# nerficg-project/faster-gaussian-splatting

Hardware: AMD Instinct MI355X
Metric: train_iters_per_sec (higher is better)
Workload: dtype f32; 1 GPU; S2: 3000000 garden-like Gaussians (SH degree 3), 1920x1080, 8 orbit views; full training iteration fwd+loss+bwd+Adam (BASELINE.json configs[2]), loss 0.8*L1+0.2*DSSIM, densification_info updated; parallelism=single GPU, n_gaussians=3000000, active_sh_bases=16, forward=one host read per pass (fgs_forward), world=1, backend=none (single process), device=cuda:0 (AMD Radeon Graphics)

## Files before the change

### faster-gaussian-splatting_amd/FasterGSCudaBackend/__init__.py

```python
from ._lib import ExtensionError, library

library()

from ._backend import RasterizerSettings
from .rasterization import (async_forward_scope, async_forward_stats, diff_rasterize, diff_rasterize_aux, live_block_stats, rasterize, rasterize_aux, set_async_forward,
                            set_live_block_handover, take_async_overflow, update_pruning_scores)
from .adam import FusedAdam
from .fused import FusedRasterizerOptimizer


from .aux_ops import add_noise, relocation_adjustment, update_3d_filter

__all__ = ['diff_rasterize', 'diff_rasterize_aux', 'rasterize', 'rasterize_aux', 'update_pruning_scores', 'RasterizerSettings', 'FusedAdam', 'update_3d_filter',
           'relocation_adjustment', 'add_noise', 'FusedRasterizerOptimizer', 'ExtensionError', 'set_async_forward', 'async_forward_stats',
           'set_live_block_handover', 'live_block_stats', 'take_async_overflow', 'async_forward_scope']
```

### faster-gaussian-splatting_amd/FasterGSCudaBackend/_backend.py

```python
from __future__ import annotations

import ctypes as C
from typing import NamedTuple, Optional, Sequence

import torch

from . import _lib


class RasterizerSettings(NamedTuple):
    w2c: torch.Tensor
    cam_position: torch.Tensor
    bg_color: torch.Tensor
    active_sh_bases: int
    width: int
    height: int
    focal_x: float
    focal_y: float
    center_x: float
    center_y: float
    near_plane: float
    far_plane: float
    proper_antialiasing: bool

# ... 191 lines not shown
        return image

    def inference_aux(self, means, scales, rotations, opacities, sh0, sh_rest, settings: RasterizerSettings, to_chw: bool,
                      clamp_output: bool, alpha: bool = True, depth_expected: bool = True, depth_median: bool = True) -> dict:
        device, S, keep, buffers, cb, st = self._forward_setup((means, scales, rotations, opacities, sh0, sh_rest), settings)
        shape = (3, settings.height, settings.width) if to_chw else (settings.height, settings.width, 3)
        out = {'rgb': torch.empty(shape, dtype=torch.float32, device=device)}
        for name, wanted in (('alpha', alpha), ('depth', depth_expected), ('depth_median', depth_median)):
            if wanted:
                out[name] = torch.empty((settings.height, settings.width), dtype=torch.float32, device=device)
        maps = [out[k].data_ptr() if k in out else None for k in ('alpha', 'depth', 'depth_median')]
        self._check(self.lib.fgs_inference_aux(_ptr(means), _ptr(scales), _ptr(rotations), _ptr(opacities), _ptr(sh0), _ptr(sh_rest),
                                               means.shape[0], C.byref(S), out['rgb'].data_ptr(), int(to_chw), int(clamp_output), *maps, cb, None,
                                               C.byref(st), _stream_of(device)), 'fgs_inference_aux')
        return out

    def pruning_scores(self, scores, means, scales, rotations, opacities, sh0, sh_rest, settings: RasterizerSettings) -> None:
        device = self._check_params((scores, means, scales, rotations, opacities, sh0, sh_rest), ('scores',) + PARAMETER_NAMES)
        if scores.numel() != means.shape[0]:
            raise RuntimeError('scores must have one entry per Gaussian')
        S, keep, buffers, cb, st = self._forward_state(settings, total_sh_rest(sh_rest), device)
        self._check(self.lib.fgs_pruning_scores(_ptr(scores), _ptr(means), _ptr(scales), _ptr(rotations), _ptr(opacities), _ptr(sh0),
                                                _ptr(sh_rest), means.shape[0], C.byref(S), cb, None, C.byref(st), _stream_of(device)),
                    'fgs_pruning_scores')

    def _scratch(self, n: int, settings: RasterizerSettings, device: torch.device) -> torch.Tensor:
        return _empty_bytes(self.lib.fgs_backward_scratch_bytes(n, int(settings.width), int(settings.height)), device)

    def _scratch_aux(self, n: int, settings: RasterizerSettings, device: torch.device) -> torch.Tensor:
        return _empty_bytes(self.lib.fgs_backward_aux_scratch_bytes(n, int(settings.width), int(settings.height)), device)

    def backward(self, densification_info, grad_image, image, means, scales, rotations, opacities, sh_rest, buffers, settings,
                 state, out: tuple | None = None, live_blocks: Optional[torch.Tensor] = None,
                 reached_blocks: Optional[torch.Tensor] = None) -> tuple:
        return self.backward_aux(densification_info, grad_image, None, None, image, None, means, scales, rotations, opacities, sh_rest, buffers, settings,
                                 state, out, live_blocks, reached_blocks)

    def backward_aux(self, densification_info, grad_image, grad_alpha, grad_depth, image, depth, means, scales, rotations, opacities, sh_rest,
                     buffers, settings, state, out: tuple | None = None, live_blocks: Optional[torch.Tensor] = None,
                     reached_blocks: Optional[torch.Tensor] = None) -> tuple:
        aux = grad_alpha is not None or grad_depth is not None
        device = self._check_params((means, scales, rotations, opacities, sh_rest), BACKWARD_PARAMETER_NAMES)
        keep: list = []
        n = means.shape[0]
        total_rest = total_sh_rest(sh_rest)
        S = self._settings(settings, total_rest, device, keep)
        grad_image = grad_image.to(dtype=torch.float32).contiguous()
        if aux:
            hw = (int(settings.height), int(settings.width))
            for name, t in (('grad_alpha', grad_alpha), ('grad_depth', grad_depth), ('depth', depth if grad_depth is not None else None)):
                if t is not None and (tuple(t.shape) != hw or t.device != device):
                    raise RuntimeError(f'{name} must be a [H,W] = {hw} tensor on the parameters\' device')
            if grad_depth is not None and depth is None:
                raise RuntimeError('backward_aux: grad_depth needs the expected-depth map of forward_aux')
            grad_alpha = grad_alpha.to(dtype=torch.float32).contiguous() if grad_alpha is not None else None
            grad_depth = grad_depth.to(dtype=torch.float32).contiguous() if grad_depth is not None else None
        depth = depth.to(dtype=torch.float32).contiguous() if grad_depth is not None else None
        grads = _gradients_out(out, gradient_shapes(n, total_rest), device)
        dens = _densification(densification_info, n, device, validate=True)
        _check_block_flags('live_blocks', live_blocks, n, device)
        _check_block_flags('reached_blocks', reached_blocks, n, device)
        scratch = (self._scratch_aux if aux else self._scratch)(n, settings, device)
        st = _lib.ForwardState(*state)
        self._check(self.lib.fgs_backward_reached(_ptr(grad_image), _ptr(image), _ptr(grad_alpha), _ptr(grad_depth), _ptr(depth), _ptr(means), _ptr(scales),
                                                  _ptr(rotations), _ptr(opacities), _ptr(sh_rest), _ptr(buffers[0]), _ptr(buffers[1]), _ptr(buffers[2]),
                                                  _ptr(buffers[3]), _ptr(grads[0]), _ptr(grads[1]), _ptr(grads[2]), _ptr(grads[3]), _ptr(grads[4]), _ptr(grads[5]),
                                                  _ptr(dens), scratch.data_ptr(), n, C.byref(S), C.byref(st), _ptr(live_blocks), _ptr(reached_blocks),
                                                  _stream_of(device)),
                    'fgs_backward_aux' if aux else 'fgs_backward')
        return grads

    def backward_adam_fused(self, densification_info, grad_image, image, params: Sequence[torch.Tensor], exp_avgs, exp_avg_sqs,
                            buffers, settings, state, step: int, lrs: Sequence[float], betas=(0.9, 0.999), eps: float = 1e-15,
                            grad_alpha=None, grad_depth=None) -> None:
        if grad_alpha is not None or grad_depth is not None:
            raise RuntimeError('backward_adam_fused takes no alpha / depth gradients: use backward_aux and an optimizer step of its own')
        device = self._check_params(tuple(params) + tuple(exp_avgs) + tuple(exp_avg_sqs), ['param/moment'] * 18)
        keep: list = []
        n = params[0].shape[0]
        S = self._settings(settings, total_sh_rest(params[2]), device, keep)
        grad_image = grad_image.to(dtype=torch.float32).contiguous()
        dens = _densification(densification_info, n, device, validate=False)
        scratch = self._scratch(n, settings, device)
        st = _lib.ForwardState(*state)
        lr_arr = (C.c_double * 6)(*[float(x) for x in lrs])
        self._check(self.lib.fgs_backward_adam_fused(_ptr(grad_image), _ptr(image), _pointer_array(params, 6), _pointer_array(exp_avgs, 6),
                                                     _pointer_array(exp_avg_sqs, 6), _ptr(buffers[0]), _ptr(buffers[1]), _ptr(buffers[2]),
                                                     _ptr(buffers[3]), _ptr(dens), scratch.data_ptr(), n, C.byref(S), C.byref(st), int(step), lr_arr,
                                                     float(betas[0]), float(betas[1]), float(eps), _stream_of(device)),
                    'fgs_backward_adam_fused')

    def adam_step(self, grad, param, exp_avg, exp_avg_sq, step: int, lr: float, beta1: float, beta2: float, eps: float) -> None:
        device = self._check_params((grad, param, exp_avg, exp_avg_sq), ('param_grad', 'param', 'exp_avg', 'exp_avg_sq'))
        self._check(self.lib.fgs_adam_step(_ptr(grad), _ptr(param), _ptr(exp_avg), _ptr(exp_avg_sq), param.numel(), int(step),
                                           float(lr), float(beta1), float(beta2), float(eps), _stream_of(device)), 'fgs_adam_step')

    def adam_step_multi(self, grads, params, exp_avgs, exp_avg_sqs, steps, lrs, beta1: float, beta2: float, eps: float,
                        live_blocks: Optional[torch.Tensor] = None, quiet_blocks: Optional[torch.Tensor] = None) -> None:
        k = len(params)
        if k == 0:
            return
# ... 277 lines not shown
```

### faster-gaussian-splatting_amd/FasterGSCudaBackend/_lib.py

```python
from __future__ import annotations

import ctypes as C
import os
from pathlib import Path

PACKAGE_ROOT = Path(__file__).resolve().parent.parent
DEFAULT_LIBRARY = PACKAGE_ROOT / 'libfgs_hip.so'

FGS_BUF_PRIMITIVE, FGS_BUF_TILE, FGS_BUF_INSTANCE, FGS_BUF_BUCKET, FGS_BUF_SCRATCH = 0, 1, 2, 3, 4


class ExtensionError(ImportError):
    """Counterpart of Framework.ExtensionError raised by the reference's package init."""


class Settings(C.Structure):
    _fields_ = [
        ('w2c', C.c_void_p), ('cam_position', C.c_void_p), ('bg_color', C.c_void_p),
        ('active_sh_bases', C.c_int32), ('total_sh_bases_rest', C.c_int32), ('width', C.c_int32), ('height', C.c_int32),
        ('focal_x', C.c_float), ('focal_y', C.c_float), ('center_x', C.c_float), ('center_y', C.c_float),
        ('near_plane', C.c_float), ('far_plane', C.c_float), ('proper_antialiasing', C.c_int32),
    ]


class ForwardState(C.Structure):
    _fields_ = [('n_visible', C.c_int32), ('n_instances', C.c_int32), ('n_buckets', C.c_int32), ('selector', C.c_int32)]


class StageTime(C.Structure):
    _fields_ = [('name', C.c_char_p), ('total_ms', C.c_double), ('calls', C.c_int64)]


class BlobEntry(C.Structure):
    _fields_ = [('name', C.c_char_p), ('offset', C.c_size_t), ('bytes', C.c_size_t)]


SPLAT_RECORD_BYTES, ACC_RECORD_BYTES = 56, 36

RESIZE_FN = C.CFUNCTYPE(C.c_void_p, C.c_void_p, C.c_int32, C.c_size_t)

_P, _I32, _I64, _F64 = C.c_void_p, C.c_int32, C.c_int64, C.c_double

_SIGNATURES = {
    'fgs_abi_version': (C.c_int32, []),
    'fgs_last_error': (C.c_char_p, []),
    'fgs_build_info': (C.c_char_p, []),
    'fgs_forward': (C.c_int32, [_P] * 6 + [_I32, C.POINTER(Settings), _P, RESIZE_FN, _P, C.POINTER(ForwardState), _P]),
    'fgs_forward_aux': (C.c_int32, [_P] * 6 + [_I32, C.POINTER(Settings), _P, _P, _P, RESIZE_FN, _P, C.POINTER(ForwardState), _P]),
    'fgs_backward_aux_scratch_bytes': (C.c_size_t, [_I32, _I32, _I32]),
    'fgs_backward_aux': (C.c_int32, [_P] * 5 + [_P] * 5 + [_P] * 4 + [_P] * 6 + [_P, _P, _I32, C.POINTER(Settings), C.POINTER(ForwardState), _P, _P]),
    'fgs_backward_reached': (C.c_int32, [_P] * 5 + [_P] * 5 + [_P] * 4 + [_P] * 6 + [_P, _P, _I32, C.POINTER(Settings), C.POINTER(ForwardState), _P, _P, _P]),
    'fgs_forward_async': (C.c_int32, [_P] * 6 + [_I32, C.POINTER(Settings), _P, _I32, RESIZE_FN, _P, C.POINTER(ForwardState), _P]),
    'fgs_forward_counts': (C.c_int32, [_P, _I32, _P, _P]),
    'fgs_backward_scratch_bytes': (C.c_size_t, [_I32, _I32, _I32]),
    'fgs_backward': (C.c_int32, [_P] * 2 + [_P] * 5 + [_P] * 4 + [_P] * 6 + [_P, _P, _I32, C.POINTER(Settings), C.POINTER(ForwardState), _P]),
    'fgs_backward_live': (C.c_int32, [_P] * 2 + [_P] * 5 + [_P] * 4 + [_P] * 6 + [_P, _P, _I32, C.POINTER(Settings), C.POINTER(ForwardState), _P, _P]),
    'fgs_inference': (C.c_int32, [_P] * 6 + [_I32, C.POINTER(Settings), _P, _I32, _I32, RESIZE_FN, _P, C.POINTER(ForwardState), _P]),
    'fgs_inference_aux': (C.c_int32, [_P] * 6 + [_I32, C.POINTER(Settings), _P, _I32, _I32, _P, _P, _P, RESIZE_FN, _P, C.POINTER(ForwardState), _P]),
    'fgs_pruning_scores': (C.c_int32, [_P] * 7 + [_I32, C.POINTER(Settings), RESIZE_FN, _P, C.POINTER(ForwardState), _P]),
    'fgs_adam_step': (C.c_int32, [_P] * 4 + [_I64, _I32, _F64, _F64, _F64, _F64, _P]),
    'fgs_adam_step_multi': (C.c_int32, [_I32] + [C.POINTER(_P)] * 4 + [C.POINTER(_I64), C.POINTER(_I32), C.POINTER(_F64), _F64, _F64, _F64, _P]),
    'fgs_adam_step_multi_live': (C.c_int32, [_I32] + [C.POINTER(_P)] * 4 + [C.POINTER(_I64), C.POINTER(_I32), C.POINTER(_F64), _F64, _F64, _F64, _P,
                                             C.POINTER(_I32), _P]),
    'fgs_adam_step_multi_quiet': (C.c_int32, [_I32] + [C.POINTER(_P)] * 4 + [C.POINTER(_I64), C.POINTER(_I32), C.POINTER(_F64), _F64, _F64, _F64, _P,
                                              C.POINTER(_I32), _P, _P]),
    'fgs_adam_quiet_scan': (C.c_int32, [_I32, C.POINTER(_P), C.POINTER(_P), C.POINTER(_I64), C.POINTER(_I32), _P, _P]),
    'fgs_backward_adam_fused': (C.c_int32, [_P] * 2 + [C.POINTER(_P)] * 3 + [_P] * 4 + [_P, _P, _I32, C.POINTER(Settings), C.POINTER(ForwardState),
                                            _I32, C.POINTER(_F64), _F64, _F64, _F64, _P]),
    'fgs_shard_preprocess': (C.c_int32, [_P] * 6 + [_I32, _I32, C.POINTER(Settings), _P, _P, RESIZE_FN, _P, _P]),
    'fgs_forward_from_records': (C.c_int32, [_P, _I32, _I32, C.POINTER(Settings), _P, RESIZE_FN, _P, C.POINTER(ForwardState), _P]),
    'fgs_backward_to_records': (C.c_int32, [_P] * 2 + [_P] * 4 + [_P, _P, _I32, C.POINTER(Settings), C.POINTER(ForwardState), _P]),
    'fgs_forward_from_shard_records': (C.c_int32, [_P, _I32, _I32, C.POINTER(_I32), _I32, C.POINTER(Settings), _P, RESIZE_FN, _P, C.POINTER(ForwardState), _P]),
    'fgs_backward_to_shard_records': (C.c_int32, [_P] * 2 + [_P] * 4 + [_P, _P, _I32, C.POINTER(_I32), _I32, C.POINTER(Settings), C.POINTER(ForwardState), _P]),
    'fgs_shard_backward_scratch_bytes': (C.c_size_t, [_I32, _I32]),
    'fgs_shard_backward': (C.c_int32, [_P, C.POINTER(_I32), _P] + [_P] * 5 + [_P] * 6 + [_P, _P, _I32, _I32, C.POINTER(Settings), _P]),
    'fgs_shard_backward_adam_fused': (C.c_int32, [_P, C.POINTER(_I32), _P] + [C.POINTER(_P)] * 3 + [_P, _P, _I32, _I32, C.POINTER(Settings), _I32,
                                                  C.POINTER(_F64), _F64, _F64, _F64, _P]),
    'fgs_blob_layout': (C.c_int32, [_I32] * 6 + [C.POINTER(BlobEntry), _I32]),
    'fgs_update_3d_filter': (C.c_int32, [_P] * 4 + [_I32, _I32, _I32] + [C.c_float] * 7 + [_P]),
    'fgs_relocation_table': (C.c_int32, [C.POINTER(C.c_float)]),
    'fgs_relocation_adjustment': (C.c_int32, [_P] * 6 + [_I32, _P]),
    'fgs_add_noise': (C.c_int32, [_P] * 5 + [_I32, C.c_float, _P]),
    'fgs_adc_scratch_bytes': (C.c_size_t, [_I32]),
    'fgs_adc_plan': (C.c_int32, [_P] * 4 + [_I32, C.c_float, C.c_float, _I32, C.c_float, C.c_float, _P, C.POINTER(_I32), _P]),
# ... 55 lines not shown
```

### faster-gaussian-splatting_amd/FasterGSCudaBackend/rasterization.py

```python
from __future__ import annotations

import math
import warnings
import weakref
from typing import Any

import torch
from torch.autograd.function import once_differentiable

from ._backend import RasterizerSettings, default_backend, gradient_shapes, total_sh_rest


_GRAD_OUT = None


def set_gradient_buffers(provider) -> None:
    global _GRAD_OUT
    _GRAD_OUT = provider


def _new_async_table() -> dict:
    return {'enabled': False, 'headroom': 1.25, 'ratio': 0.0, 'overflows': 0, 'per_view': {}, 'pending': {}, 'step_invalid': False, 'ticket': 0}


# ... 9 lines not shown

    def __enter__(self):
        global _ASYNC
        self._outer = _ASYNC
        _ASYNC = _ASYNC_SCOPES.setdefault(self.name, _new_async_table())
        return self

    def __exit__(self, *exc):
        global _ASYNC
        _ASYNC = self._outer

    @staticmethod
    def drop(name) -> None:
        if name is not None:
            _ASYNC_SCOPES.pop(name, None)

_LIVE = {'enabled': True, 'slots': {}, 'matched': 0, 'missed': 0}
_LIVE_MAX_SLOTS = 8
_ALIGN_FLOATS = 64


def set_live_block_handover(enabled: bool) -> None:
    _LIVE['enabled'] = bool(enabled)
    clear_live_blocks()


def live_block_stats() -> dict:
    return {'matched': _LIVE['matched'], 'missed': _LIVE['missed']}


def clear_live_blocks(owned=None) -> None:
    if owned is None:
        _LIVE['slots'].clear()
        return
    for t in owned:
        _LIVE['slots'].pop(t.data_ptr(), None)


def _gradient_arena(shapes, device):
    numels = [math.prod(sh) for sh in shapes]
    offsets, total = [], 0
    for numel in numels:
        offsets.append(total)
        total += (numel + _ALIGN_FLOATS - 1) // _ALIGN_FLOATS * _ALIGN_FLOATS
    arena = torch.empty(max(total, 1), dtype=torch.float32, device=device)
    return arena, tuple(arena[off:off + numel].view(sh) for sh, off, numel in zip(shapes, offsets, numels))


def match_live_blocks(gradients, owned=None) -> 'torch.Tensor | None':
    slots = _LIVE['slots']
    keys = list(slots) if owned is None else [t.data_ptr() for t in owned if t.data_ptr() in slots]
    if not keys or len(gradients) == 0:
        return None
    first = gradients[0].data_ptr()
    key = next((k for k in keys if any(address == first for address, _ in slots[k]['views'])), keys[0])
    slot = slots.pop(key)
    arena, flags, views, version = slot['arena'], slot['flags'], slot['views'], slot['version']
    by_address = {address: shape for address, shape in views if address != 0}
    seen = set()
    for g in gradients:
        shape = by_address.get(g.data_ptr())
        if (shape is None or g.data_ptr() in seen or tuple(g.shape) != shape or g.dtype != torch.float32 or not g.is_contiguous()
                or g.device != arena.device or g._version != version):
            _LIVE['missed'] += 1
            return None
        seen.add(g.data_ptr())
    _LIVE['matched'] += 1
    return flags


def set_async_forward(enabled: bool, headroom: float = 1.25) -> None:
    _ASYNC.update(enabled=bool(enabled), headroom=float(headroom))
    if not enabled:
        _ASYNC.update(ratio=0.0, per_view={}, pending={}, step_invalid=False)


def async_forward_stats() -> dict:
    return {'enabled': _ASYNC['enabled'], 'headroom': _ASYNC['headroom'], 'ratio': _ASYNC['ratio'], 'overflows': _ASYNC['overflows'],
            'views': len(_ASYNC['per_view']), 'unchecked_passes': len(_ASYNC['pending'])}


def take_async_overflow(owned=None) -> bool:
    if owned is None:
        marked, _ASYNC['step_invalid'] = _ASYNC['step_invalid'], False
        return bool(marked)
    mine = {a for t in owned for a in _addresses(t)}
    for table in _ASYNC_SCOPES.values():
        if table['step_invalid'] and not mine.isdisjoint(table['step_invalid']):
            table['step_invalid'] = False
# ... 95 lines not shown
        ctx.save_for_backward(res.image, means, scales, rotations, opacities, sh_coefficients_rest, *res.buffers)
        ctx.densification_info = densification_info
        ctx.mark_non_differentiable(densification_info)
        return res.image

    @staticmethod
    @once_differentiable
    def backward(ctx: Any, grad_image: torch.Tensor):
        image, means, scales, rotations, opacities, sh_rest, *buffers = ctx.saved_tensors
        state, A = ctx.buffer_state, ctx.async_table
        if ctx.async_check is not None:
            host, event, key, ticket = ctx.async_check
            A['pending'].pop(ticket, None)
            if event is not None:
                event.synchronize()
            n = means.shape[0]
            _record_ratio(A, key, ctx.rasterizer_settings.w2c, int(host[1]) / max(n, 1))
            if int(host[2]) != 0:
                A['overflows'] += 1
                warnings.warn(f'FasterGS async forward: {int(host[1])} instances exceeded the capacity {state[1]} of this pass: its image was '
                              f'incomplete, so this backward pass returns zero gradients and FusedAdam.step skips the step (the view is rendered with the '
                              f'right capacity next time)', RuntimeWarning)
                clear_live_blocks([means])
                A['step_invalid'] = frozenset(a for t in (means, scales, rotations, opacities, sh_rest) for a in _addresses(t)) | frozenset(ctx.sh0_addresses)
                if _GRAD_OUT is not None:
                    zeros = tuple(_GRAD_OUT())
                    for z in zeros:
                        z.zero_()
                else:
                    zeros = tuple(torch.zeros(sh, dtype=torch.float32, device=means.device) for sh in gradient_shapes(n, total_sh_rest(sh_rest)))
                return (*zeros, None, None)
        n = means.shape[0]
        handover = _LIVE['enabled'] and _GRAD_OUT is None and n > 0
        if handover:
            arena, out = _gradient_arena(gradient_shapes(n, total_sh_rest(sh_rest)), means.device)
            live, flags = torch.empty((2, (n + 63) // 64), dtype=torch.uint8, device=means.device)
        else:
            clear_live_blocks([means])
            out, live, flags = (_GRAD_OUT() if _GRAD_OUT is not None else None), None, None
        grads = default_backend().backward(ctx.densification_info, grad_image, image, means, scales, rotations, opacities, sh_rest,
                                           buffers, ctx.rasterizer_settings, state, out=out, live_blocks=live, reached_blocks=flags)
        if handover:
            slots = _LIVE['slots']
            slots.pop(means.data_ptr(), None)
            slots[means.data_ptr()] = {'arena': arena, 'version': arena._version, 'flags': flags,
                                       'views': tuple((v.data_ptr() if v.numel() else 0, tuple(v.shape)) for v in out)}
            while len(slots) > _LIVE_MAX_SLOTS:
                del slots[next(iter(slots))]
        del out
        return (*grads, None, None)


def diff_rasterize(means: torch.Tensor, scales: torch.Tensor, rotations: torch.Tensor, opacities: torch.Tensor,
                   sh_coefficients_0: torch.Tensor, sh_coefficients_rest: torch.Tensor, densification_info: torch.Tensor,
                   rasterizer_settings: RasterizerSettings) -> torch.Tensor:
    return _Rasterize.apply(means, scales, rotations, opacities, sh_coefficients_0, sh_coefficients_rest, densification_info,
                            rasterizer_settings)


class _RasterizeAux(torch.autograd.Function):

    @staticmethod
    def forward(ctx: Any, means, scales, rotations, opacities, sh_coefficients_0, sh_coefficients_rest, densification_info,
                rasterizer_settings: RasterizerSettings, alpha: bool, depth: bool):
        _require_gpu(means)
        res = default_backend().forward_aux(means, scales, rotations, opacities, sh_coefficients_0, sh_coefficients_rest, rasterizer_settings, alpha, depth)
        ctx.rasterizer_settings = rasterizer_settings
        ctx.buffer_state = res.state
        ctx.has_depth = res.depth is not None
        ctx.set_materialize_grads(False)
        shape = (rasterizer_settings.height, rasterizer_settings.width)
        a = res.alpha if res.alpha is not None else means.new_empty(shape)
        d = res.depth if res.depth is not None else means.new_empty(shape)
        ctx.save_for_backward(res.image, d, means, scales, rotations, opacities, sh_coefficients_rest, *res.buffers)
# ... 65 lines not shown
```

### faster-gaussian-splatting_amd/csrc/api.hip

```cpp
#include "fgs_host.h"
#include <cstdarg>
#include <cstdio>
#include <vector>

using namespace fgs;
namespace {
thread_local char g_error[512] = "";

const char* const kStageNames[ST_COUNT] = {"preprocess", "depth_sort", "offsets_scan", "create_instances", "tile_sort", "extract_ranges",
                                           "bucket_scan", "blend_forward", "stage_pixels", "blend_backward", "preprocess_backward",
                                           "sh_rest_backward", "adam", "l1_dssim_loss", "shard_records", "fused_backward_adam"};
struct StageRecord { int stage; hipEvent_t start, stop; };
struct Profiler {
    bool enabled = false;
    int only = -1;
    std::vector<StageRecord> records;
    std::vector<hipEvent_t> pool;
    hipEvent_t get() {
        if (!pool.empty()) { hipEvent_t e = pool.back(); pool.pop_back(); return e; }
        hipEvent_t e = nullptr;
        if (hipEventCreate(&e) != hipSuccess) return nullptr;
        return e;
    }
};
// ... 310 lines not shown
                          void* primitive_buffers, void* tile_buffers, void* instance_buffers, void* bucket_buffers,
                          float* grad_means, float* grad_scales, float* grad_rotations, float* grad_opacities,
                          float* grad_sh_coefficients_0, float* grad_sh_coefficients_rest,
                          float* densification_info, void* scratch,
                          int32_t n_primitives, const fgs_settings* settings, const fgs_forward_state* state, uint8_t* live_blocks, void* stream_) {
    return fgs_backward_aux(grad_image, image, nullptr, nullptr, nullptr, means, scales, rotations, opacities, sh_coefficients_rest, primitive_buffers,
                            tile_buffers, instance_buffers, bucket_buffers, grad_means, grad_scales, grad_rotations, grad_opacities, grad_sh_coefficients_0,
                            grad_sh_coefficients_rest, densification_info, scratch, n_primitives, settings, state, live_blocks, stream_);
}

int32_t fgs_backward_aux(const float* grad_image, const float* image, const float* grad_alpha, const float* grad_depth, const float* depth_expected,
                         const float* means, const float* scales, const float* rotations, const float* opacities,
                         const float* sh_coefficients_rest,
                         void* primitive_buffers, void* tile_buffers, void* instance_buffers, void* bucket_buffers,
                         float* grad_means, float* grad_scales, float* grad_rotations, float* grad_opacities,
                         float* grad_sh_coefficients_0, float* grad_sh_coefficients_rest,
                         float* densification_info, void* scratch,
                         int32_t n_primitives, const fgs_settings* settings, const fgs_forward_state* state, uint8_t* live_blocks, void* stream_) {
    return fgs_backward_reached(grad_image, image, grad_alpha, grad_depth, depth_expected, means, scales, rotations, opacities, sh_coefficients_rest,
                                primitive_buffers, tile_buffers, instance_buffers, bucket_buffers, grad_means, grad_scales, grad_rotations, grad_opacities,
                                grad_sh_coefficients_0, grad_sh_coefficients_rest, densification_info, scratch, n_primitives, settings, state, live_blocks,
                                nullptr, stream_);
}

int32_t fgs_backward_reached(const float* grad_image, const float* image, const float* grad_alpha, const float* grad_depth, const float* depth_expected,
                             const float* means, const float* scales, const float* rotations, const float* opacities,
                             const float* sh_coefficients_rest,
                             void* primitive_buffers, void* tile_buffers, void* instance_buffers, void* bucket_buffers,
                             float* grad_means, float* grad_scales, float* grad_rotations, float* grad_opacities,
                             float* grad_sh_coefficients_0, float* grad_sh_coefficients_rest,
                             float* densification_info, void* scratch,
                             int32_t n_primitives, const fgs_settings* settings, const fgs_forward_state* state, uint8_t* live_blocks,
                             uint8_t* reached_blocks, void* stream_) {
    const bool with_maps = grad_alpha != nullptr || grad_depth != nullptr;
    BackwardPlan P;
    if (int rc = plan_backward(P, {primitive_buffers, tile_buffers, instance_buffers, bucket_buffers, scratch}, n_primitives, settings, state, with_maps)) return rc;
    if (!grad_image || !image) return fail(FGS_ERR_INVALID_ARGUMENT, "NULL image / grad_image");
    if (grad_depth && !(state->selector & kStateDepthCheckpoints))
        return fail(FGS_ERR_INVALID_ARGUMENT, "grad_depth needs the depth checkpoints that fgs_forward_aux writes: these buffers were filled by a forward pass without them");
    if (grad_depth && !depth_expected) return fail(FGS_ERR_INVALID_ARGUMENT, "grad_depth without depth_expected (the map fgs_forward_aux returned)");
    if (n_primitives == 0) return FGS_OK;
    if (!means || !scales || !rotations || !opacities || !grad_means || !grad_scales || !grad_rotations || !grad_opacities || !grad_sh_coefficients_0)
        return fail(FGS_ERR_INVALID_ARGUMENT, "NULL parameter / gradient tensor");
    hipStream_t stream = static_cast<hipStream_t>(stream_);
    if (with_maps) { if (int rc = run_blend_backward_aux(P, grad_image, image, grad_alpha, grad_depth, depth_expected, means, stream)) return rc; }
    else if (int rc = run_blend_backward(P, grad_image, image, stream)) return rc;

    PreprocessBackwardArgs a{};
    ShRestArgs sh{};
    fill_backward_args(a, sh, {means, scales, rotations, opacities, nullptr, sh_coefficients_rest}, static_cast<uint32_t>(n_primitives), 1, *settings);
    set_backward_view(a, sh, 0, backward_view(*settings, P.geo, P.pb.n_touched, nullptr, P.pb.acc, P.sc.view_dir));
    if (grad_depth) a.view[0].acc_z = P.sc.acc_z;
    a.grad_means = grad_means; a.grad_scales = grad_scales; a.grad_rotations = grad_rotations; a.grad_opacities = grad_opacities;
    a.grad_sh0 = grad_sh_coefficients_0; a.densification_info = densification_info;
    if (settings->total_sh_bases_rest > 0 && !grad_sh_coefficients_rest) return fail(FGS_ERR_INVALID_ARGUMENT, "NULL grad_sh_coefficients_rest");
    sh.grad_sh_rest = grad_sh_coefficients_rest;
    if (g_fused_single_kernel) {
        StageScope t(ST_PREPROCESS_BACKWARD, stream);
        a.live_blocks = live_blocks;
        a.reached_blocks = reached_blocks;
        FGS_HIP(launch_backward_gradients(a, sh, stream));
    } else {
        if (live_blocks != nullptr) FGS_HIP(hipMemsetAsync(live_blocks, 1, (static_cast<size_t>(n_primitives) + 63) / 64, stream));
        if (reached_blocks != nullptr) FGS_HIP(hipMemsetAsync(reached_blocks, 1, (static_cast<size_t>(n_primitives) + 63) / 64, stream));
        { StageScope t(ST_PREPROCESS_BACKWARD, stream); FGS_HIP(launch_preprocess_backward(false, a, stream)); }
        if (settings->total_sh_bases_rest > 0) { StageScope t(ST_SH_REST_BACKWARD, stream); FGS_HIP(launch_sh_rest_backward(false, sh, stream)); }
    }
    if (grad_depth) { StageScope t(ST_PREPROCESS_BACKWARD, stream); FGS_HIP(launch_depth_mean_gradient(P.sc.acc_z, P.pb.n_touched, settings->w2c, grad_means, static_cast<uint32_t>(n_primitives), stream)); }
    return FGS_OK;
}

int32_t fgs_backward(const float* grad_image, const float* image,
                     const float* means, const float* scales, const float* rotations, const float* opacities,
                     const float* sh_coefficients_rest,
                     void* primitive_buffers, void* tile_buffers, void* instance_buffers, void* bucket_buffers,
                     float* grad_means, float* grad_scales, float* grad_rotations, float* grad_opacities,
                     float* grad_sh_coefficients_0, float* grad_sh_coefficients_rest,
                     float* densification_info, void* scratch,
                     int32_t n_primitives, const fgs_settings* settings, const fgs_forward_state* state, void* stream) {
    return fgs_backward_live(grad_image, image, means, scales, rotations, opacities, sh_coefficients_rest, primitive_buffers, tile_buffers,
                             instance_buffers, bucket_buffers, grad_means, grad_scales, grad_rotations, grad_opacities, grad_sh_coefficients_0,
                             grad_sh_coefficients_rest, densification_info, scratch, n_primitives, settings, state, nullptr, stream);
}

int32_t fgs_backward_adam_fused(const float* grad_image, const float* image,
                                float* const* params, float* const* exp_avgs, float* const* exp_avg_sqs,
                                void* primitive_buffers, void* tile_buffers, void* instance_buffers, void* bucket_buffers,
                                float* densification_info, void* scratch,
                                int32_t n_primitives, const fgs_settings* settings, const fgs_forward_state* state,
                                int32_t step, const double* lrs, double beta1, double beta2, double eps, void* stream_) {
    BackwardPlan P;
    if (int rc = plan_backward(P, {primitive_buffers, tile_buffers, instance_buffers, bucket_buffers, scratch}, n_primitives, settings, state)) return rc;
    const FusedAdam adam{params, exp_avgs, exp_avg_sqs, step, lrs, beta1, beta2, eps};
// ... 61 lines not shown
```

### faster-gaussian-splatting_amd/csrc/fgs_kernels.h

```cpp
#pragma once
#include <hip/hip_runtime.h>
#include <atomic>
#include <cmath>
#include <cstddef>
#include <cstdint>
#include "fgs_config.h"
#include "fgs_math.h"

namespace fgs {

struct PreprocessArgs {
    const float* means; const float* scales; const float* rotations; const float* opacities;
    const float* sh0; const float* sh_rest;
    PrimRec* rec; uint32_t* n_touched;
    uint32_t* depth_keys; uint32_t* prim_idx;
    uint4* foot;
    uint32_t* counters;
    uint32_t* huge_list;
    uint32_t* hot_list;
    uint2* ranges; uint32_t n_tiles;
    float* acc;
    uint32_t n;
    int seq_tiles;
    int count_appended;
// ... 105 lines not shown
    const float* depth;
    const float* ckpt_d;
    float4* pixaux;
    const float* means; const float* w2c;
    float* acc_z;
    float* acc_z_hot;
    uint32_t clear_z_f4;
};
struct BlendBackwardDepthArgs { BlendBackwardArgs blend; BlendDepthPart d; };
hipError_t launch_stage_pixels_depth(const BlendBackwardDepthArgs& a, hipStream_t s);
hipError_t launch_blend_backward_depth(const BlendBackwardDepthArgs& a, hipStream_t s);
hipError_t launch_depth_mean_gradient(const float* acc_z, const uint32_t* n_touched, const float* w2c, float* grad_means, uint32_t n, hipStream_t s);

struct AdamHyper { float step_size, beta1, beta2, eps, bc2_sqrt_rcp; };

struct BackwardView {
    CameraArgs cam;
    const uint32_t* n_touched;
    const float* acc;
    const uint32_t* slot;
    float* view_dir;
    const float* acc_z;
};
struct PreprocessBackwardArgs {
    const float* means; const float* scales; const float* rotations; const float* opacities; const float* sh_rest;
    float* grad_means; float* grad_scales; float* grad_rotations; float* grad_opacities; float* grad_sh0;
    float* densification_info;
    uint32_t n;
    int accumulate;
    int n_views; BackwardView view[kMaxBatchViews];
    float* p[5]; float* m[5]; float* v[5]; AdamHyper h[5];
    uint8_t* live_blocks;
    uint8_t* reached_blocks;
    int vector_ok;
};
hipError_t launch_preprocess_backward(bool fused_adam, const PreprocessBackwardArgs& a, hipStream_t s);

struct ShRestView { const float* view_dir; const uint32_t* n_touched; const float* acc; const uint32_t* slot; };
struct ShRestArgs {
    int n_views; ShRestView view[kMaxBatchViews];
    float* grad_sh_rest;
    float* p; float* m; float* v; AdamHyper h;
    uint32_t n; uint32_t total_sh_rest; uint32_t active_sh_bases;
    int accumulate;
};
hipError_t launch_sh_rest_backward(bool fused_adam, const ShRestArgs& a, hipStream_t s);
hipError_t launch_fused_backward_adam(const PreprocessBackwardArgs& a, const ShRestArgs& sh, hipStream_t s);
hipError_t launch_backward_gradients(const PreprocessBackwardArgs& a, const ShRestArgs& sh, hipStream_t s);

struct AdamGroup { const float* grad; float* param; float* exp_avg; float* exp_avg_sq; int64_t n; AdamHyper h; uint32_t first_block;
                   uint32_t row_len; };
struct AdamArgs { AdamGroup g[8]; int n_groups; uint32_t total_blocks; int reverse; const uint8_t* live_blocks; uint8_t* quiet_blocks; };
hipError_t launch_adam(const AdamArgs& a, hipStream_t s);
struct AdamQuietScanArgs { const float* m[8]; const float* v[8]; uint32_t row_len[8]; int n_groups; uint32_t rows; uint8_t* quiet_out; };
hipError_t launch_adam_quiet_scan(const AdamQuietScanArgs& a, hipStream_t s);

struct LossArgs {
    const float* image; const float* target;
    float* sums;
    float* grad;
    float* d_mu; float* d_m11; float* d_m12;
    float* partials;
    int width, height;
    float lambda_l1, lambda_dssim;
    const float* upstream;
};
// ... 61 lines not shown
```

### faster-gaussian-splatting_amd/csrc/preprocess_backward.hip

```cpp
#include "fgs_adam.h"
#include <type_traits>

namespace fgs {

constexpr int kGroupWidth[5] = {3, 3, 1, 3, 4};
constexpr int kGroupOffset[5] = {0, 3, 6, 7, 10};

template <bool MULTI> __device__ __forceinline__ void sum_into(float& dst, const float v) { dst = MULTI ? dst + v : v; }

#ifndef FGS_K12_RECORD_EARLY
#define FGS_K12_RECORD_EARLY 0
#endif
template <bool FUSED, bool MULTI, bool KEEP_DIR>
__device__ __forceinline__ bool gaussian_backward(const PreprocessBackwardArgs& a, const unsigned i, const float (&st_p)[14],
                                                  float (&grad)[14], float (&dir)[3], float (&gcol_out)[3], bool& reached) {
    const size_t n = a.n;
    float g_mean[3] = {0.0f, 0.0f, 0.0f}, g_scale[3] = {0.0f, 0.0f, 0.0f}, g_rot[4] = {0.0f, 0.0f, 0.0f, 0.0f};
    float g_op[1] = {0.0f}, g_sh0[3] = {0.0f, 0.0f, 0.0f};
    bool visible = false;
    reached = false;
    float m[3] = {0.0f, 0.0f, 0.0f}, s[3] = {0.0f, 0.0f, 0.0f}, q[4] = {0.0f, 0.0f, 0.0f, 0.0f};
    const int n_views = MULTI ? a.n_views : 1;
    const Camera cam0 = load_camera(a.view[0].cam);
    for (int vw = 0; vw < n_views; ++vw) {
// ... 343 lines not shown
    if (w.R == 0) return;

    const bool any_reached = wave_ballot(reached) != 0;
    if (any_reached) {
        put_sh_factors(slice, w.lane, reached, dir, gcol, sh.active_sh_bases);
        wave_lds_fence();
    }

    float* const P = sh.p + w.base; float* const M = sh.m + w.base; float* const V = sh.v + w.base;
    for (uint32_t e0 = 4u * w.lane; e0 < w.count; e0 += 4u * kWave * kFusedUnroll) {
        AdamPiece piece[kFusedUnroll];
        bool full[kFusedUnroll];
#pragma unroll
        for (int u = 0; u < kFusedUnroll; ++u) {
            const uint32_t e = e0 + 4u * kWave * static_cast<uint32_t>(u);
            full[u] = e + 4u <= w.count && a.vector_ok != 0;
            if (full[u]) piece[u].load(P + e, M + e, V + e);
        }
#pragma unroll
        for (int u = 0; u < kFusedUnroll; ++u) {
            const uint32_t e = e0 + 4u * kWave * static_cast<uint32_t>(u);
            if (full[u])
                piece[u].step(P + e, M + e, V + e, any_reached ? sh_rest_gradient_piece<RT>(slice, e, w.R) : make_float4(0.0f, 0.0f, 0.0f, 0.0f), sh.h);
            else if (e < w.count)
                adam_scalar_tail(P, M, V, e, w.count < e + 4u ? w.count : e + 4u, sh.h,
                                 [&](const uint32_t j) { return any_reached ? sh_rest_gradient_at<RT>(slice, j, w.R) : 0.0f; });
        }
    }
}

#ifndef FGS_K12_NT_STORES
#define FGS_K12_NT_STORES 1
#endif
template <int RT>
__global__ void __launch_bounds__(256) backward_gradients_kernel(const PreprocessBackwardArgs a, const ShRestArgs sh) {
    __shared__ __attribute__((aligned(16))) float s_grad[256 / kWave][kWave * 15 * 3];
    const WaveBlock w = wave_block<RT>(a.n, sh.total_sh_rest);
    if (w.first >= a.n) return;
    const uint32_t i = w.first + w.lane;
    const bool in_range = i < a.n;
    float grad[14], dir[3] = {0.0f, 0.0f, 0.0f}, gcol[3] = {0.0f, 0.0f, 0.0f};
    const float unused[14] = {};
    bool visible = false, reached = false;
    if (in_range) {
        visible = gaussian_backward<false, false, true>(a, i, unused, grad, dir, gcol, reached);
        float* const outs[5] = {a.grad_means, a.grad_sh0, a.grad_opacities, a.grad_scales, a.grad_rotations};
#pragma unroll
        for (int grp = 0; grp < 5; ++grp)
#pragma unroll
            for (int k = 0; k < kGroupWidth[grp]; ++k) {
#if FGS_K12_NT_STORES >= 2
                __builtin_nontemporal_store(grad[kGroupOffset[grp] + k], outs[grp] + (size_t)i * kGroupWidth[grp] + k);
#else
                outs[grp][(size_t)i * kGroupWidth[grp] + k] = grad[kGroupOffset[grp] + k];
#endif
            }
    }
    float* const slice = s_grad[w.wv];
    const bool any_visible = wave_ballot(visible) != 0, any_reached = wave_ballot(reached) != 0;
    if (a.live_blocks != nullptr && w.lane == 0) a.live_blocks[w.first >> 6] = any_visible ? 1 : 0;
    if (a.reached_blocks != nullptr && w.lane == 0) a.reached_blocks[w.first >> 6] = any_reached ? 1 : 0;
    if (w.R == 0) return;
    if (any_reached) {
        float B[15];
        lane_sh_basis(B, reached && sh.active_sh_bases > 1, dir[0], dir[1], dir[2], sh.active_sh_bases);
        float* const mine = slice + w.lane * w.R * 3u;
#pragma unroll
        for (int k = 0; k < 15; ++k)
            if (static_cast<uint32_t>(k) < w.R) { mine[3 * k] = B[k] * gcol[0]; mine[3 * k + 1] = B[k] * gcol[1]; mine[3 * k + 2] = B[k] * gcol[2]; }
        wave_lds_fence();
    }
    float* const out = sh.grad_sh_rest + w.base;
    for (uint32_t e = 4u * w.lane; e < w.count; e += 4u * kWave) {
        if (e + 4u <= w.count && a.vector_ok) {
            const float4 g = any_reached ? *reinterpret_cast<const float4*>(slice + e) : make_float4(0.0f, 0.0f, 0.0f, 0.0f);
#if FGS_K12_NT_STORES
            store_float4_nt(out + e, g);
#else
            *reinterpret_cast<float4*>(out + e) = g;
#endif
        } else {
            for (uint32_t j = e; j < w.count && j < e + 4u; ++j) out[j] = any_reached ? slice[j] : 0.0f;
        }
    }
}

static bool aligned16(const void* p) { return (reinterpret_cast<uintptr_t>(p) & 15u) == 0; }

template <class Launch> static hipError_t dispatch_sh_rest(const uint32_t total_sh_rest, Launch launch) {
    if (total_sh_rest > 15) return hipErrorInvalidValue;
    if (total_sh_rest == 15) launch(std::integral_constant<int, 15>());
    else launch(std::integral_constant<int, 0>());
    return hipGetLastError();
}
// ... 182 lines not shown
```

### include/fgs_hip.h

```cpp
#ifndef FGS_HIP_H
#define FGS_HIP_H

#include <stddef.h>
#include <stdint.h>

#ifdef __cplusplus
extern "C" {
#endif

#define FGS_ABI_VERSION 3

typedef enum fgs_status {
    FGS_OK = 0,
    FGS_ERR_INVALID_ARGUMENT = -1,
    FGS_ERR_ALLOC = -2,
    FGS_ERR_HIP = -3,
    FGS_ERR_INTERNAL = -4
} fgs_status;

typedef struct fgs_settings {
    const float* w2c;
    const float* cam_position;
    const float* bg_color;
    int32_t active_sh_bases;
// ... 34 lines not shown
                     float* densification_info, void* scratch,
                     int32_t n_primitives, const fgs_settings* settings, const fgs_forward_state* state, void* stream);
int32_t fgs_backward_live(const float* grad_image, const float* image,
                          const float* means, const float* scales, const float* rotations, const float* opacities,
                          const float* sh_coefficients_rest,
                          void* primitive_buffers, void* tile_buffers, void* instance_buffers, void* bucket_buffers,
                          float* grad_means, float* grad_scales, float* grad_rotations, float* grad_opacities,
                          float* grad_sh_coefficients_0, float* grad_sh_coefficients_rest,
                          float* densification_info, void* scratch,
                          int32_t n_primitives, const fgs_settings* settings, const fgs_forward_state* state, uint8_t* live_blocks, void* stream);

int32_t fgs_forward_aux(const float* means, const float* scales, const float* rotations, const float* opacities,
                        const float* sh_coefficients_0, const float* sh_coefficients_rest, int32_t n_primitives,
                        const fgs_settings* settings, float* image, float* alpha, float* depth_expected,
                        fgs_resize_fn resize, void* resize_user, fgs_forward_state* state_out, void* stream);
size_t fgs_backward_aux_scratch_bytes(int32_t n_primitives, int32_t width, int32_t height);
int32_t fgs_backward_aux(const float* grad_image, const float* image, const float* grad_alpha, const float* grad_depth, const float* depth_expected,
                         const float* means, const float* scales, const float* rotations, const float* opacities,
                         const float* sh_coefficients_rest,
                         void* primitive_buffers, void* tile_buffers, void* instance_buffers, void* bucket_buffers,
                         float* grad_means, float* grad_scales, float* grad_rotations, float* grad_opacities,
                         float* grad_sh_coefficients_0, float* grad_sh_coefficients_rest,
                         float* densification_info, void* scratch,
                         int32_t n_primitives, const fgs_settings* settings, const fgs_forward_state* state, uint8_t* live_blocks, void* stream);
int32_t fgs_backward_reached(const float* grad_image, const float* image, const float* grad_alpha, const float* grad_depth, const float* depth_expected,
                             const float* means, const float* scales, const float* rotations, const float* opacities,
                             const float* sh_coefficients_rest,
                             void* primitive_buffers, void* tile_buffers, void* instance_buffers, void* bucket_buffers,
                             float* grad_means, float* grad_scales, float* grad_rotations, float* grad_opacities,
                             float* grad_sh_coefficients_0, float* grad_sh_coefficients_rest,
                             float* densification_info, void* scratch,
                             int32_t n_primitives, const fgs_settings* settings, const fgs_forward_state* state, uint8_t* live_blocks,
                             uint8_t* reached_blocks, void* stream);

int32_t fgs_forward_async(const float* means, const float* scales, const float* rotations, const float* opacities,
                          const float* sh_coefficients_0, const float* sh_coefficients_rest, int32_t n_primitives,
                          const fgs_settings* settings, float* image, int32_t instance_capacity, fgs_resize_fn resize, void* resize_user,
                          fgs_forward_state* state_out, void* stream);
int32_t fgs_forward_counts(const void* primitive_buffers, int32_t n_primitives, int32_t* host_out, void* stream);

int32_t fgs_inference(const float* means, const float* scales, const float* rotations, const float* opacities,
                      const float* sh_coefficients_0, const float* sh_coefficients_rest, int32_t n_primitives,
                      const fgs_settings* settings, float* image, int32_t to_chw, int32_t clamp_output,
                      fgs_resize_fn resize, void* resize_user, fgs_forward_state* state_out, void* stream);

int32_t fgs_inference_aux(const float* means, const float* scales, const float* rotations, const float* opacities,
                          const float* sh_coefficients_0, const float* sh_coefficients_rest, int32_t n_primitives,
                          const fgs_settings* settings, float* image, int32_t to_chw, int32_t clamp_output,
                          float* alpha, float* depth_expected, float* depth_median,
                          fgs_resize_fn resize, void* resize_user, fgs_forward_state* state_out, void* stream);

int32_t fgs_pruning_scores(float* scores, const float* means, const float* scales, const float* rotations, const float* opacities,
                           const float* sh_coefficients_0, const float* sh_coefficients_rest, int32_t n_primitives,
                           const fgs_settings* settings, fgs_resize_fn resize, void* resize_user, fgs_forward_state* state_out, void* stream);

int32_t fgs_adam_step(const float* grad, float* param, float* exp_avg, float* exp_avg_sq, int64_t n_elements,
                      int32_t step, double lr, double beta1, double beta2, double eps, void* stream);

int32_t fgs_adam_step_multi(int32_t n_groups, const float* const* grads, float* const* params, float* const* exp_avgs,
                            float* const* exp_avg_sqs, const int64_t* n_elements, const int32_t* steps, const double* lrs,
                            double beta1, double beta2, double eps, void* stream);
int32_t fgs_adam_step_multi_live(int32_t n_groups, const float* const* grads, float* const* params, float* const* exp_avgs,
                                 float* const* exp_avg_sqs, const int64_t* n_elements, const int32_t* steps, const double* lrs,
                                 double beta1, double beta2, double eps, const uint8_t* live_blocks, const int32_t* floats_per_gaussian,
                                 void* stream);
int32_t fgs_adam_step_multi_quiet(int32_t n_groups, const float* const* grads, float* const* params, float* const* exp_avgs,
// ... 107 lines not shown
```

Before: 669.9 iters/s (1 view each, whole job).

## Recycle gradient arenas and skip zero-writes for blocks already zero from prior pass

Keeps the gradient arena from the previous backward pass as a spare and reuses it when nothing else still references it and its version is unchanged. The reached-block flags of that pass are passed to the preprocess-backward kernel as prior_blocks. A wave whose block was not reached before and is not reached now skips storing the per-Gaussian gradients, since those entries already hold zeros (checked by sampling the first element). This cuts write bandwidth for the many unreached Gaussians of a 3M-Gaussian model. The cost is a reuse scheme that relies on storage reference counts and version tracking, which is fragile if the arena is modified externally in ways those checks miss.

After: 699.1 iters/s (1 view each, whole job), median of 6. 1.04x the previous value.

```diff
diff --git a/faster-gaussian-splatting_amd/FasterGSCudaBackend/__init__.py b/faster-gaussian-splatting_amd/FasterGSCudaBackend/__init__.py
--- a/faster-gaussian-splatting_amd/FasterGSCudaBackend/__init__.py
+++ b/faster-gaussian-splatting_amd/FasterGSCudaBackend/__init__.py
@@ -3,8 +3,8 @@
 library()
 
 from ._backend import RasterizerSettings
-from .rasterization import (async_forward_scope, async_forward_stats, diff_rasterize, diff_rasterize_aux, live_block_stats, rasterize, rasterize_aux, set_async_forward,
-                            set_live_block_handover, take_async_overflow, update_pruning_scores)
+from .rasterization import (async_forward_scope, async_forward_stats, diff_rasterize, diff_rasterize_aux, gradient_recycling_stats, live_block_stats, rasterize,
+                            rasterize_aux, set_async_forward, set_gradient_recycling, set_live_block_handover, take_async_overflow, update_pruning_scores)
 from .adam import FusedAdam
 from .fused import FusedRasterizerOptimizer
 
@@ -13,4 +13,4 @@
 
 __all__ = ['diff_rasterize', 'diff_rasterize_aux', 'rasterize', 'rasterize_aux', 'update_pruning_scores', 'RasterizerSettings', 'FusedAdam', 'update_3d_filter',
            'relocation_adjustment', 'add_noise', 'FusedRasterizerOptimizer', 'ExtensionError', 'set_async_forward', 'async_forward_stats',
-           'set_live_block_handover', 'live_block_stats', 'take_async_overflow', 'async_forward_scope']
+           'set_live_block_handover', 'live_block_stats', 'set_gradient_recycling', 'gradient_recycling_stats', 'take_async_overflow', 'async_forward_scope']
diff --git a/faster-gaussian-splatting_amd/FasterGSCudaBackend/_backend.py b/faster-gaussian-splatting_amd/FasterGSCudaBackend/_backend.py
--- a/faster-gaussian-splatting_amd/FasterGSCudaBackend/_backend.py
+++ b/faster-gaussian-splatting_amd/FasterGSCudaBackend/_backend.py
@@ -247,13 +247,13 @@
 
     def backward(self, densification_info, grad_image, image, means, scales, rotations, opacities, sh_rest, buffers, settings,
                  state, out: tuple | None = None, live_blocks: Optional[torch.Tensor] = None,
-                 reached_blocks: Optional[torch.Tensor] = None) -> tuple:
+                 reached_blocks: Optional[torch.Tensor] = None, prior_blocks: Optional[torch.Tensor] = None) -> tuple:
         return self.backward_aux(densification_info, grad_image, None, None, image, None, means, scales, rotations, opacities, sh_rest, buffers, settings,
-                                 state, out, live_blocks, reached_blocks)
+                                 state, out, live_blocks, reached_blocks, prior_blocks)
 
     def backward_aux(self, densification_info, grad_image, grad_alpha, grad_depth, image, depth, means, scales, rotations, opacities, sh_rest,
                      buffers, settings, state, out: tuple | None = None, live_blocks: Optional[torch.Tensor] = None,
-                     reached_blocks: Optional[torch.Tensor] = None) -> tuple:
+                     reached_blocks: Optional[torch.Tensor] = None, prior_blocks: Optional[torch.Tensor] = None) -> tuple:
         aux = grad_alpha is not None or grad_depth is not None
         device = self._check_params((means, scales, rotations, opacities, sh_rest), BACKWARD_PARAMETER_NAMES)
         keep: list = []
@@ -275,13 +275,14 @@
         dens = _densification(densification_info, n, device, validate=True)
         _check_block_flags('live_blocks', live_blocks, n, device)
         _check_block_flags('reached_blocks', reached_blocks, n, device)
+        _check_block_flags('prior_blocks', prior_blocks, n, device)
         scratch = (self._scratch_aux if aux else self._scratch)(n, settings, device)
         st = _lib.ForwardState(*state)
-        self._check(self.lib.fgs_backward_reached(_ptr(grad_image), _ptr(image), _ptr(grad_alpha), _ptr(grad_depth), _ptr(depth), _ptr(means), _ptr(scales),
-                                                  _ptr(rotations), _ptr(opacities), _ptr(sh_rest), _ptr(buffers[0]), _ptr(buffers[1]), _ptr(buffers[2]),
-                                                  _ptr(buffers[3]), _ptr(grads[0]), _ptr(grads[1]), _ptr(grads[2]), _ptr(grads[3]), _ptr(grads[4]), _ptr(grads[5]),
-                                                  _ptr(dens), scratch.data_ptr(), n, C.byref(S), C.byref(st), _ptr(live_blocks), _ptr(reached_blocks),
-                                                  _stream_of(device)),
+        self._check(self.lib.fgs_backward_recycled(_ptr(grad_image), _ptr(image), _ptr(grad_alpha), _ptr(grad_depth), _ptr(depth), _ptr(means), _ptr(scales),
+                                                   _ptr(rotations), _ptr(opacities), _ptr(sh_rest), _ptr(buffers[0]), _ptr(buffers[1]), _ptr(buffers[2]),
+                                                   _ptr(buffers[3]), _ptr(grads[0]), _ptr(grads[1]), _ptr(grads[2]), _ptr(grads[3]), _ptr(grads[4]), _ptr(grads[5]),
+                                                   _ptr(dens), scratch.data_ptr(), n, C.byref(S), C.byref(st), _ptr(live_blocks), _ptr(reached_blocks),
+                                                   _ptr(prior_blocks), _stream_of(device)),
                     'fgs_backward_aux' if aux else 'fgs_backward')
         return grads
 
diff --git a/faster-gaussian-splatting_amd/FasterGSCudaBackend/_lib.py b/faster-gaussian-splatting_amd/FasterGSCudaBackend/_lib.py
--- a/faster-gaussian-splatting_amd/FasterGSCudaBackend/_lib.py
+++ b/faster-gaussian-splatting_amd/FasterGSCudaBackend/_lib.py
@@ -50,6 +50,7 @@
     'fgs_backward_aux_scratch_bytes': (C.c_size_t, [_I32, _I32, _I32]),
     'fgs_backward_aux': (C.c_int32, [_P] * 5 + [_P] * 5 + [_P] * 4 + [_P] * 6 + [_P, _P, _I32, C.POINTER(Settings), C.POINTER(ForwardState), _P, _P]),
     'fgs_backward_reached': (C.c_int32, [_P] * 5 + [_P] * 5 + [_P] * 4 + [_P] * 6 + [_P, _P, _I32, C.POINTER(Settings), C.POINTER(ForwardState), _P, _P, _P]),
+    'fgs_backward_recycled': (C.c_int32, [_P] * 5 + [_P] * 5 + [_P] * 4 + [_P] * 6 + [_P, _P, _I32, C.POINTER(Settings), C.POINTER(ForwardState), _P, _P, _P, _P]),
     'fgs_forward_async': (C.c_int32, [_P] * 6 + [_I32, C.POINTER(Settings), _P, _I32, RESIZE_FN, _P, C.POINTER(ForwardState), _P]),
     'fgs_forward_counts': (C.c_int32, [_P, _I32, _P, _P]),
     'fgs_backward_scratch_bytes': (C.c_size_t, [_I32, _I32, _I32]),
diff --git a/faster-gaussian-splatting_amd/FasterGSCudaBackend/rasterization.py b/faster-gaussian-splatting_amd/FasterGSCudaBackend/rasterization.py
--- a/faster-gaussian-splatting_amd/FasterGSCudaBackend/rasterization.py
+++ b/faster-gaussian-splatting_amd/FasterGSCudaBackend/rasterization.py
@@ -65,19 +65,65 @@
 def clear_live_blocks(owned=None) -> None:
     if owned is None:
         _LIVE['slots'].clear()
+        _RECYCLE['spares'].clear()
         return
     for t in owned:
-        _LIVE['slots'].pop(t.data_ptr(), None)
-
-
-def _gradient_arena(shapes, device):
+        _retire(_LIVE['slots'].pop(t.data_ptr(), None))
+
+
+def _gradient_arena(shapes, device, arena=None):
     numels = [math.prod(sh) for sh in shapes]
     offsets, total = [], 0
     for numel in numels:
         offsets.append(total)
         total += (numel + _ALIGN_FLOATS - 1) // _ALIGN_FLOATS * _ALIGN_FLOATS
-    arena = torch.empty(max(total, 1), dtype=torch.float32, device=device)
+    if arena is None:
+        arena = torch.empty(max(total, 1), dtype=torch.float32, device=device)
     return arena, tuple(arena[off:off + numel].view(sh) for sh, off, numel in zip(shapes, offsets, numels))
+
+
+_RECYCLE = {'enabled': True, 'spares': {}, 'recycled': 0, 'fresh': 0, 'baseline': {}}
+_RECYCLE_MAX_SPARES = 2
+_STORAGE_USE_COUNT = getattr(torch._C, '_storage_Use_Count', None)
+
+
+def set_gradient_recycling(enabled: bool) -> None:
+    _RECYCLE['enabled'] = bool(enabled)
+    _RECYCLE['spares'].clear()
+
+
+def gradient_recycling_stats() -> dict:
+    return {'recycled': _RECYCLE['recycled'], 'fresh': _RECYCLE['fresh']}
+
+
+def _storage_references(t: torch.Tensor) -> int:
+    return _STORAGE_USE_COUNT(t.untyped_storage()._cdata)
+
+
+def _retire(slot) -> None:
+    if slot is None or not _RECYCLE['enabled'] or _STORAGE_USE_COUNT is None:
+        return
+    spares, arena = _RECYCLE['spares'], slot['arena']
+    key = (arena.device, tuple(shape for _, shape in slot['views']))
+    spares.pop(key, None)
+    spares[key] = {'arena': arena, 'version': slot['version'], 'flags': slot['flags']}
+    while len(spares) > _RECYCLE_MAX_SPARES:
+        del spares[next(iter(spares))]
+
+
+def _take_spare(shapes, device):
+    spare = _RECYCLE['spares'].pop((device, tuple(tuple(sh) for sh in shapes)), None)
+    if spare is None or not _RECYCLE['enabled'] or _STORAGE_USE_COUNT is None:
+        return None
+    if device.type == 'cuda' and torch.cuda.is_current_stream_capturing():
+        return None
+    arena = spare['arena']
+    baseline = _RECYCLE['baseline'].get(device.type)
+    if baseline is None:
+        baseline = _RECYCLE['baseline'][device.type] = _storage_references(torch.empty(1, dtype=torch.float32, device=device))
+    if arena._version != spare['version'] or _storage_references(arena) != baseline:
+        return None
+    return spare
 
 
 def match_live_blocks(gradients, owned=None) -> 'torch.Tensor | None':
@@ -88,6 +134,7 @@
     first = gradients[0].data_ptr()
     key = next((k for k in keys if any(address == first for address, _ in slots[k]['views'])), keys[0])
     slot = slots.pop(key)
+    _retire(slot)
     arena, flags, views, version = slot['arena'], slot['flags'], slot['views'], slot['version']
     by_address = {address: shape for address, shape in views if address != 0}
     seen = set()
@@ -249,14 +296,21 @@
                 return (*zeros, None, None)
         n = means.shape[0]
         handover = _LIVE['enabled'] and _GRAD_OUT is None and n > 0
+        prior = None
         if handover:
-            arena, out = _gradient_arena(gradient_shapes(n, total_sh_rest(sh_rest)), means.device)
+            shapes = gradient_shapes(n, total_sh_rest(sh_rest))
+            spare = _take_spare(shapes, means.device)
+            if spare is not None:
+                prior = spare['flags']
+            _RECYCLE['recycled' if spare is not None else 'fresh'] += 1
+            arena, out = _gradient_arena(shapes, means.device, None if spare is None else spare['arena'])
+            del spare
             live, flags = torch.empty((2, (n + 63) // 64), dtype=torch.uint8, device=means.device)
         else:
             clear_live_blocks([means])
             out, live, flags = (_GRAD_OUT() if _GRAD_OUT is not None else None), None, None
         grads = default_backend().backward(ctx.densification_info, grad_image, image, means, scales, rotations, opacities, sh_rest,
-                                           buffers, ctx.rasterizer_settings, state, out=out, live_blocks=live, reached_blocks=flags)
+                                           buffers, ctx.rasterizer_settings, state, out=out, live_blocks=live, reached_blocks=flags, prior_blocks=prior)
         if handover:
             slots = _LIVE['slots']
             slots.pop(means.data_ptr(), None)
diff --git a/faster-gaussian-splatting_amd/csrc/api.hip b/faster-gaussian-splatting_amd/csrc/api.hip
--- a/faster-gaussian-splatting_amd/csrc/api.hip
+++ b/faster-gaussian-splatting_amd/csrc/api.hip
@@ -366,6 +366,25 @@
                              float* densification_info, void* scratch,
                              int32_t n_primitives, const fgs_settings* settings, const fgs_forward_state* state, uint8_t* live_blocks,
                              uint8_t* reached_blocks, void* stream_) {
+    return fgs_backward_recycled(grad_image, image, grad_alpha, grad_depth, depth_expected, means, scales, rotations, opacities, sh_coefficients_rest,
+                                 primitive_buffers, tile_buffers, instance_buffers, bucket_buffers, grad_means, grad_scales, grad_rotations, grad_opacities,
+                                 grad_sh_coefficients_0, grad_sh_coefficients_rest, densification_info, scratch, n_primitives, settings, state, live_blocks,
+                                 reached_blocks, nullptr, stream_);
+}
+
+int32_t fgs_backward_recycled(const float* grad_image, const float* image, const float* grad_alpha, const float* grad_depth, const float* depth_expected,
+                              const float* means, const float* scales, const float* rotations, const float* opacities,
+                              const float* sh_coefficients_rest,
+                              void* primitive_buffers, void* tile_buffers, void* instance_buffers, void* bucket_buffers,
+                              float* grad_means, float* grad_scales, float* grad_rotations, float* grad_opacities,
+                              float* grad_sh_coefficients_0, float* grad_sh_coefficients_rest,
+                              float* densification_info, void* scratch,
+                              int32_t n_primitives, const fgs_settings* settings, const fgs_forward_state* state, uint8_t* live_blocks,
+                              uint8_t* reached_blocks, const uint8_t* prior_blocks, void* stream_) {
+    if (prior_blocks != nullptr && reached_blocks == nullptr)
+        return fail(FGS_ERR_INVALID_ARGUMENT, "prior_blocks without reached_blocks: the caller could not make the promise again for the next pass");
+    if (prior_blocks != nullptr && (prior_blocks == reached_blocks || prior_blocks == live_blocks))
+        return fail(FGS_ERR_INVALID_ARGUMENT, "prior_blocks aliases %s: the pass reads the one while it writes the other", prior_blocks == reached_blocks ? "reached_blocks" : "live_blocks");
     const bool with_maps = grad_alpha != nullptr || grad_depth != nullptr;
     BackwardPlan P;
     if (int rc = plan_backward(P, {primitive_buffers, tile_buffers, instance_buffers, bucket_buffers, scratch}, n_primitives, settings, state, with_maps)) return rc;
@@ -393,6 +412,7 @@
         StageScope t(ST_PREPROCESS_BACKWARD, stream);
         a.live_blocks = live_blocks;
         a.reached_blocks = reached_blocks;
+        a.prior_blocks = prior_blocks;
         FGS_HIP(launch_backward_gradients(a, sh, stream));
     } else {
         if (live_blocks != nullptr) FGS_HIP(hipMemsetAsync(live_blocks, 1, (static_cast<size_t>(n_primitives) + 63) / 64, stream));
diff --git a/faster-gaussian-splatting_amd/csrc/fgs_kernels.h b/faster-gaussian-splatting_amd/csrc/fgs_kernels.h
--- a/faster-gaussian-splatting_amd/csrc/fgs_kernels.h
+++ b/faster-gaussian-splatting_amd/csrc/fgs_kernels.h
@@ -161,6 +161,7 @@
     float* p[5]; float* m[5]; float* v[5]; AdamHyper h[5];
     uint8_t* live_blocks;
     uint8_t* reached_blocks;
+    const uint8_t* prior_blocks;
     int vector_ok;
 };
 hipError_t launch_preprocess_backward(bool fused_adam, const PreprocessBackwardArgs& a, hipStream_t s);
diff --git a/faster-gaussian-splatting_amd/csrc/preprocess_backward.hip b/faster-gaussian-splatting_amd/csrc/preprocess_backward.hip
--- a/faster-gaussian-splatting_amd/csrc/preprocess_backward.hip
+++ b/faster-gaussian-splatting_amd/csrc/preprocess_backward.hip
@@ -399,18 +399,33 @@
 #ifndef FGS_K12_NT_STORES
 #define FGS_K12_NT_STORES 1
 #endif
+__device__ __forceinline__ bool block_promised_zero(const PreprocessBackwardArgs& a, const ShRestArgs& sh, const WaveBlock& w) {
+    if (a.prior_blocks == nullptr) return false;
+    const size_t first = wave_uniform(w.first);
+    if (a.prior_blocks[first >> 6] != 0) return false;
+    const float s0 = a.grad_means[3u * first], s1 = a.grad_sh0[3u * first], s2 = a.grad_opacities[first], s3 = a.grad_scales[3u * first],
+                s4 = a.grad_rotations[4u * first], s5 = w.R > 0 ? sh.grad_sh_rest[first * w.R * 3u] : 0.0f;
+    return s0 == 0.0f && s1 == 0.0f && s2 == 0.0f && s3 == 0.0f && s4 == 0.0f && s5 == 0.0f;
+}
+
 template <int RT>
 __global__ void __launch_bounds__(256) backward_gradients_kernel(const PreprocessBackwardArgs a, const ShRestArgs sh) {
     __shared__ __attribute__((aligned(16))) float s_grad[256 / kWave][kWave * 15 * 3];
     const WaveBlock w = wave_block<RT>(a.n, sh.total_sh_rest);
     if (w.first >= a.n) return;
+    const bool promised_zero = block_promised_zero(a, sh, w);
     const uint32_t i = w.first + w.lane;
     const bool in_range = i < a.n;
     float grad[14], dir[3] = {0.0f, 0.0f, 0.0f}, gcol[3] = {0.0f, 0.0f, 0.0f};
     const float unused[14] = {};
     bool visible = false, reached = false;
+    if (in_range) visible = gaussian_backward<false, false, true>(a, i, unused, grad, dir, gcol, reached);
+    float* const slice = s_grad[w.wv];
+    const bool any_visible = wave_ballot(visible) != 0, any_reached = wave_ballot(reached) != 0;
+    if (a.live_blocks != nullptr && w.lane == 0) a.live_blocks[w.first >> 6] = any_visible ? 1 : 0;
+    if (a.reached_blocks != nullptr && w.lane == 0) a.reached_blocks[w.first >> 6] = any_reached ? 1 : 0;
+    if (!any_reached && promised_zero) return;
     if (in_range) {
-        visible = gaussian_backward<false, false, true>(a, i, unused, grad, dir, gcol, reached);
         float* const outs[5] = {a.grad_means, a.grad_sh0, a.grad_opacities, a.grad_scales, a.grad_rotations};
 #pragma unroll
         for (int grp = 0; grp < 5; ++grp)
@@ -423,10 +438,6 @@
 #endif
             }
     }
-    float* const slice = s_grad[w.wv];
-    const bool any_visible = wave_ballot(visible) != 0, any_reached = wave_ballot(reached) != 0;
-    if (a.live_blocks != nullptr && w.lane == 0) a.live_blocks[w.first >> 6] = any_visible ? 1 : 0;
-    if (a.reached_blocks != nullptr && w.lane == 0) a.reached_blocks[w.first >> 6] = any_reached ? 1 : 0;
     if (w.R == 0) return;
     if (any_reached) {
         float B[15];
diff --git a/include/fgs_hip.h b/include/fgs_hip.h
--- a/include/fgs_hip.h
+++ b/include/fgs_hip.h
@@ -90,6 +90,15 @@
                              float* densification_info, void* scratch,
                              int32_t n_primitives, const fgs_settings* settings, const fgs_forward_state* state, uint8_t* live_blocks,
                              uint8_t* reached_blocks, void* stream);
+int32_t fgs_backward_recycled(const float* grad_image, const float* image, const float* grad_alpha, const float* grad_depth, const float* depth_expected,
+                              const float* means, const float* scales, const float* rotations, const float* opacities,
+                              const float* sh_coefficients_rest,
+                              void* primitive_buffers, void* tile_buffers, void* instance_buffers, void* bucket_buffers,
+                              float* grad_means, float* grad_scales, float* grad_rotations, float* grad_opacities,
+                              float* grad_sh_coefficients_0, float* grad_sh_coefficients_rest,
+                              float* densification_info, void* scratch,
+                              int32_t n_primitives, const fgs_settings* settings, const fgs_forward_state* state, uint8_t* live_blocks,
+                              uint8_t* reached_blocks, const uint8_t* prior_blocks, void* stream);
 
 int32_t fgs_forward_async(const float* means, const float* scales, const float* rotations, const float* opacities,
                           const float* sh_coefficients_0, const float* sh_coefficients_rest, int32_t n_primitives,
```
